# nikopj/FluxMPI.jl

Hardware: AMD Instinct MI355X
Metric: images/sec ResNet50 Lux.jl DDP at 1/2/4/8 MI355X; scaling efficiency (higher is better)
Workload: dtype bf16; 1 GPU; model=ResNet50, global_batch=256, per_gpu_batch=256, image_size=224, parallelism=dp1, optimizer=adam, conv=hybrid, norm=fused, memory_format=channels_last, backend=rccl, miopen_find=True, hip_graph=False, tunableop=False, kernel_choices=shipped, loss_finite=True, communicate=False

## Files before the change

csrc/api.h:

```cpp
#pragma once
#include <hip/hip_runtime.h>
#include <cstdint>
#include <vector>

namespace fluxmpi {

void mt_copy(const std::vector<uintptr_t>& src, const std::vector<uintptr_t>& dst,
             const std::vector<int64_t>& numel, int in_dtype, int out_dtype, double scale,
             hipStream_t stream);

void mt_fill(const std::vector<uintptr_t>& dst, const std::vector<int64_t>& numel, int dtype,
             double value, hipStream_t stream);

void mt_sumsq(const std::vector<uintptr_t>& src, const std::vector<int64_t>& numel, int dtype,
              float* out, hipStream_t stream);

struct SrHyper {
  uint64_t seed;
  uint32_t stream;
  uint32_t step;
  const uint32_t* dev_step;
  const int64_t* offsets = nullptr;
  size_t n_offsets = 0;
};
// ... 187 lines not shown
  const void* res;
  int64_t ldr;
  const void* bnb_x;
  const float* bnb_w;
  const float* bnb_b;
  const float* bnb_mean;
  const float* bnb_inv;
  const uint8_t* bnb_mask;
  int bnb_rm;
  int conv_h = 0, conv_w = 0, conv_c = 0;
  int engine = 0;
  const uint8_t* res_mask = nullptr;
  int res_sub_h = 0, res_sub_w = 0;
  int a_sub_h = 0, a_sub_w = 0;
  int conv_s = 1;
};
void gemm_bf16(const GemmProblem& g, hipStream_t stream);
void conv3bn3_bwd(const GemmProblem& g, hipStream_t stream);
void conv3ds_bwd(const void* dy, const uint8_t* relu_mask, const void* c3, const void* cds, const float* w,
                 const float* save_mean, const float* save_invstd, const float* sum_dy, const float* sum_dy_xhat,
                 const float* w2, const float* save_mean2, const float* save_invstd2, const float* sum_dy2,
                 const float* sum_dy_xhat2, const void* a2, const void* x, const void* wt3, const void* wtds,
                 void* d_a2, void* d_xside, float* ws3, float* wsds, int64_t P, int slabs, hipStream_t stream);
bool gemm_glds_supported(const GemmProblem& g);
void gemm_glds(const GemmProblem& g, hipStream_t stream);
void gemm_wgrad(const void* a, const void* b, float* ws, int64_t lda, int64_t ldb, int64_t M, int64_t N, int64_t K,
                int splits, int conv_h, int conv_w, int conv_c, hipStream_t stream, int variant = 0, int b_sub = 0);
void transpose_filters(const std::vector<uintptr_t>& src, const std::vector<uintptr_t>& dst,
                       const std::vector<int>& co, const std::vector<int>& ci, const std::vector<int>& taps,
                       hipStream_t stream);
void gemm_splitk_reduce(const float* ws, int splits, int64_t n, void* out, int out_dtype, hipStream_t stream);
void gemm_splitk_reduce_seg(const float* ws, int splits, int64_t n, int64_t seg, void* out0, void* out1, void* out2,
                            int out_dtype, hipStream_t stream);
bool wgrad256_supported(int64_t M, int64_t N, int64_t K, int64_t lda, int64_t ldb);
int wgrad256_actual_splits(int64_t K, int splits);
void wgrad256_set_variant(int v);
void gemm_wgrad256(const void* a, const void* b, float* ws, int64_t lda, int64_t ldb, int64_t M, int64_t N, int64_t K,
                   int splits, hipStream_t stream);
bool gemm_nt_supported(int64_t M, int64_t N, int64_t K, int64_t lda, int64_t ldb, int64_t ldc);
bool gemm_nt_conv_supported(int64_t pixels, int64_t C, int64_t Cout);
int gemm_nt_colpart_rows(int64_t M);
void gemm_nt_set_split(int min_ktiles);
int gemm_nt_get_split();
void gemm_nt(const void* a, const void* b, void* c, void* c2, const void* bias, int bias_f32, const void* h,
             float* colpart, float* stats, int64_t lda, int64_t ldb, int64_t ldc, int64_t M, int64_t N, int64_t K,
             int epi, hipStream_t stream);
// ... 67 lines not shown
```

csrc/bindings.cpp:

```cpp
#include <array>
#include <type_traits>
#include <pybind11/pybind11.h>
#include <pybind11/stl.h>

#include "api.h"
#include "comm/rccl_comm.h"

namespace py = pybind11;
using namespace fluxmpi;

template <typename T> using Py = std::conditional_t<std::is_pointer_v<T>, uintptr_t, T>;

template <typename T> T ptr(Py<T> v) {
  if constexpr (std::is_pointer_v<T>) return reinterpret_cast<T>(v);
  else return v;
}

template <typename T> std::array<T, 3> ptr3(const std::array<uintptr_t, 3>& v) {
  return {ptr<T>(v[0]), ptr<T>(v[1]), ptr<T>(v[2])};
}

template <typename R, typename... A> auto raw(R (*fn)(A...)) {
  return [fn](Py<A>... a) -> R { return fn(ptr<A>(a)...); };
}
// ... 107 lines not shown
PYBIND11_MODULE(_C_sr, m) {
  m.doc() = "fluxmpi_amd native library: stochastic rounding of the fused optimisers' bf16 stores";
  m.def("mt_adam", with_sr(&py_mt_adam), ADAM_ARGS, NO_SKIP, SR_ARGS);
  m.def("mt_sgd", with_sr(&py_mt_sgd), SGD_ARGS, NO_SKIP, SR_ARGS);
  m.def("mt_rule", with_sr(&py_mt_rule), RULE_ARGS, NO_SKIP, SR_ARGS);
  m.def(
      "mt_stochastic_round",
      [](Ptrs dst, Ptrs src, const std::vector<int64_t>& numel, uintptr_t dev_skip, uintptr_t stream, uint64_t seed,
         uint32_t sr_stream, uint32_t step, uintptr_t dev_step, const std::vector<int64_t>& offsets) {
        mt_stochastic_round(dst, src, numel, sr_hyper(seed, sr_stream, step, dev_step, offsets),
                            ptr<const int32_t*>(dev_skip), ptr<hipStream_t>(stream));
      },
      py::arg("dst"), py::arg("src"), py::arg("numel"), py::arg("dev_skip"), py::arg("stream"), SR_ARGS);
  m.def("sr_advance", raw(&sr_advance), py::arg("block"), py::arg("dev_skip"), py::arg("stream"));
}

PYBIND11_MODULE(_C_c3ds, m) {
  m.doc() = "fluxmpi_amd native library: one-pass backward around the dual BatchNorm of a downsample block";
  m.def("conv3ds_bwd", raw(&conv3ds_bwd), py::arg("dy"), py::arg("mask"), py::arg("c3"), py::arg("cds"), py::arg("w"),
        py::arg("mean"), py::arg("inv"), py::arg("sum_dy"), py::arg("sum_dy_xhat"), py::arg("w2"), py::arg("mean2"),
        py::arg("inv2"), py::arg("sum_dy2"), py::arg("sum_dy_xhat2"), py::arg("a2"), py::arg("x"), py::arg("wt3"),
        py::arg("wtds"), py::arg("d_a2"), py::arg("d_xside"), py::arg("ws3"), py::arg("wsds"), py::arg("P"),
        py::arg("slabs"), py::arg("stream"));
}

PYBIND11_MODULE(_C_aug, m) {
  m.doc() = "fluxmpi_amd native library: crop, flip, normalise, mixup / cutmix of a uint8 batch in one pass";
  m.def(
      "augment_batch",
      [](uintptr_t in, uintptr_t out, int64_t B, int H, int W, int h, int w, int C, int dtype, uint64_t seed,
         uint32_t aug_stream, uint32_t step, int64_t sample_offset, int mode, std::array<int, 4> box, float lam, int pad,
         int fill, int crop_center, int flip, std::array<float, 3> a, std::array<float, 3> b, uintptr_t dev_block,
         uintptr_t stream) {
        AugHyper hy{seed, aug_stream, step, sample_offset, mode, box[0], box[1], box[2], box[3], lam, pad, fill,
                    crop_center, flip, {a[0], a[1], a[2]}, {b[0], b[1], b[2]}, ptr<const uint32_t*>(dev_block)};
        augment_batch(ptr<const void*>(in), ptr<void*>(out), B, H, W, h, w, C, dtype, hy, ptr<hipStream_t>(stream));
      },
      py::arg("input"), py::arg("out"), py::arg("B"), py::arg("H"), py::arg("W"), py::arg("h"), py::arg("w"),
      py::arg("C"), py::arg("dtype"), py::arg("seed"), py::arg("aug_stream"), py::arg("step"),
      py::arg("sample_offset"), py::arg("mode"), py::arg("box"), py::arg("lam"), py::arg("pad"), py::arg("fill"),
      py::arg("crop_center"), py::arg("flip"), py::arg("a"), py::arg("b"), py::arg("dev_block"), py::arg("stream"));
  m.def(
      "aug_block_set",
      [](uintptr_t block, uint32_t step, int mode, std::array<int, 4> box, float lam, uintptr_t stream) {
        aug_block_set(ptr<void*>(block), step, mode, box[0], box[1], box[2], box[3], lam, ptr<hipStream_t>(stream));
      },
// ... 207 lines not shown
```

fluxmpi_amd/_build.py:

```python
from __future__ import annotations

import concurrent.futures as cf
import glob
import os
import re
import shutil
import subprocess
import sys
import sysconfig

ROOT = os.path.dirname(os.path.dirname(os.path.abspath(__file__)))
CSRC = os.path.join(ROOT, "csrc")
BUILD = os.path.join(ROOT, "build", "native")
ROCM = os.environ.get("ROCM_PATH", "/opt/rocm")
ARCH = os.environ.get("FLUXMPI_ARCH", "gfx950")


def _ext_suffix() -> str:
    return sysconfig.get_config_var("EXT_SUFFIX") or ".so"


def output_path() -> str:
    return os.path.join(ROOT, "fluxmpi_amd", "_C" + _ext_suffix())

# ... 9 lines not shown


def _torch_lib() -> str:
    import importlib.util

    spec = importlib.util.find_spec("torch")
    return os.path.join(os.path.dirname(spec.origin), "lib")


def _tool(name: str) -> str:
    for cand in (os.path.join(ROCM, "bin", name), os.path.join(ROCM, "llvm", "bin", name), shutil.which(name)):
        if cand and os.path.exists(cand):
            return cand
    raise FileNotFoundError(f"{name} not found (ROCM_PATH={ROCM})")


def _obj_for(src: str) -> str:
    rel = os.path.relpath(src, CSRC).replace(os.sep, "__")
    return os.path.join(BUILD, rel + ".o")


_NO_SLP = ["-fno-slp-vectorize"]
EXTRA_FLAGS = {f: _NO_SLP for f in ("gemm_nt.hip", "attention.hip", "gemm_glds.hip", "gemm.hip", "conv3x3n.hip",
                                        "wgrad3x3n.hip", "linbwd.hip", "conv3bn3_bwd.hip", "conv3ds_bwd.hip")}


NO_SCRATCH = ("conv3bn3_bwd.hip", "conv3ds_bwd.hip")


def _check_no_scratch(src: str, remarks: str) -> None:
    sizes = [int(m) for m in re.findall(r"ScratchSize \[bytes/lane\]: (\d+)", remarks)]
    if not sizes:
        raise RuntimeError(f"{src}: the compiler printed no kernel resource usage to check for scratch")
    if any(sizes):
        raise RuntimeError(f"{src}: a kernel spills to scratch ({max(sizes)} bytes/lane); it must not\n{remarks}")


def _compile_cmd(src: str, obj: str) -> list[str]:
    import pybind11

    common = ["-O3", "-fPIC", "-std=c++17", "-I", CSRC, "-Wall", "-Wno-unused-function",
              "-Wno-unused-variable", "-Wno-unused-but-set-variable"]
    if src.endswith(".hip"):
        return [_tool("hipcc"), f"--offload-arch={ARCH}", "-c", src, "-o", obj, *common,
                "-munsafe-fp-atomics", *EXTRA_FLAGS.get(os.path.basename(src), []),
                *(["-Rpass-analysis=kernel-resource-usage"] if os.path.basename(src) in NO_SCRATCH else [])]
    inc = [f"-I{pybind11.get_include()}", f"-I{sysconfig.get_paths()['include']}", f"-I{ROCM}/include"]
    return [_tool("amdclang++"), "-D__HIP_PLATFORM_AMD__=1", "-c", src, "-o", obj, *common, *inc,
            "-fvisibility=hidden"]

# ... 54 lines not shown
```

fluxmpi_amd/models/resnet.py:

```python
from __future__ import annotations

import os

import torch
import torch.nn as nn
import torch.nn.functional as F

from ..ops.linear import Linear

STEM = os.environ.get("FLUXMPI_STEM", "ours")


class Conv1x1(nn.Module):

    def __init__(self, cin: int, cout: int, stride: int = 1):
        super().__init__()
        self.stride = stride
        self.weight = nn.Parameter(torch.empty(cout, cin, 1, 1))
        nn.init.kaiming_normal_(self.weight, mode="fan_out", nonlinearity="relu")

    def forward(self, x):
        if self.stride != 1:
            x = x[:, :, ::self.stride, ::self.stride]
        n, c, h, w = x.shape
# ... 87 lines not shown
                    c1 = fb.conv1x1_stats(x, self.conv1.weight, link)
                    a1 = fb.bn_from_stats(c1, self.bn1, relu=True)
                cds = None
                c3ds = False
                if self.downsample is None:
                    identity = x
                elif fused_ds:
                    ds = self.downsample
                    dual = fb.dual_bn_ok(x, ds[0].out_channels, self.bn3, ds[1])
                    ds_stats = dual and fb.ds_forward_is_ours(x, ds[0].weight, ds[0].stride[0])
                    c3ds = self.hybrid and fb.conv3ds_ok(x, self.conv2, self.conv3, self.bn3, ds[0], ds[1])
                    identity = None
                    if not c3ds:
                        identity = fb.conv1x1_downsample(x, ds[0].weight, ds[0].stride[0],
                                                         link if isinstance(link, fb.SideGradLink) else None,
                                                         ours_stats=ds_stats)
                        if dual:
                            cds, identity = identity, None
                        else:
                            identity = ds[1](identity)
                else:
                    identity = self.downsample(x)
                if self.hybrid:
                    if fb.conv3x3_supported(a1, self.conv2):
                        ours = fb.conv3x3_forward_is_ours(a1, self.conv2.weight)
                        c2 = fb.conv3x3(a1, self.conv2.weight, with_stats=True)
                        a2 = fb.bn_from_stats(c2, self.bn2, relu=True, stats_ready=ours)
                    elif fb.conv3x3_s2_supported(a1, self.conv2):
                        ours = fb.conv3x3_s2_forward_is_ours(a1, self.conv2.weight)
                        c2 = fb.conv3x3_s2(a1, self.conv2.weight, with_stats=ours)
                        a2 = fb.bn_from_stats(c2, self.bn2, relu=True, stats_ready=ours)
                    else:
                        a2 = self.bn2(self.conv2(a1), relu=True)
                    o3 = fb.conv1x1_forward_is_ours(a2, self.conv3.weight)
                    if self.downsample is None and fb.conv3bn3_ok(a2, self.conv3, self.bn3, identity, link):
                        return fb.conv3_bn3_relu(a2, self.conv3, self.bn3, identity, link, ours_fwd=o3)
                    if c3ds:
                        return fb.conv3ds_bn_relu(a2, self.conv3, self.bn3, x, ds[0], ds[1], link, ours3=o3,
                                                  ours_ds=ds_stats)
                    c3 = fb.conv1x1_hybrid(a2, self.conv3.weight, None, ours_stats=o3)
                else:
                    c2 = fb.conv3x3(a1, self.conv2.weight) if fb.conv3x3_supported(a1, self.conv2) else self.conv2(a1)
                    c3 = fb.bn_relu_conv1x1(c2, self.bn2, self.conv3.weight)
                if cds is not None:
                    out = fb.dual_bn_relu(c3, self.bn3, cds, self.downsample[1],
                                          stats_ready=o3 if self.hybrid else True, ds_stats_ready=ds_stats)
                elif self.hybrid and not o3:
                    out = self.bn3(c3, relu=True, residual=identity, link=link if self.downsample is None else None)
                elif self.hybrid:
                    out = fb.bn_from_stats(c3, self.bn3, relu=True, residual=identity, stats_ready=True,
                                           link=link if self.downsample is None else None)
                else:
                    out = fb.bn_from_stats(c3, self.bn3, relu=True, residual=identity,
                                           link=link if self.downsample is None else None)
                return out
        identity = x if self.downsample is None else self.downsample(x)
        if self.fused:
            out = self.bn1(self.conv1(x), relu=True)
            out = self.bn2(self.conv2(out), relu=True)
            return self.bn3(self.conv3(out), relu=True, residual=identity)
        out = F.relu(self.bn1(self.conv1(x)))
        out = F.relu(self.bn2(self.conv2(out)))
        out = self.bn3(self.conv3(out))
# ... 94 lines not shown
```

fluxmpi_amd/ops/_ext.py:

```python
from __future__ import annotations

import importlib
import importlib.util
import os

import torch

from ..utils.errors import NativeExtensionError

_MOD = None
_TRIED = False
_ERR: Exception | None = None


def _try_import():
    global _MOD, _TRIED, _ERR
    if _TRIED:
        return _MOD
    _TRIED = True
    try:
        _MOD = importlib.import_module("fluxmpi_amd._C")
    except Exception as e:
        _MOD = None
        _ERR = e
# ... 39 lines not shown
            raise NativeExtensionError(
                f"fluxmpi_amd.{name} ({what} of {C.__file__}) failed to load: {e!r}. "
                "Rebuild: `python -c 'import fluxmpi_amd; fluxmpi_amd.build()'`.") from e
        _EXTRA[name] = mod
    return _EXTRA[name]


def scale():
    return _extra("_C_scale", "the loss-scaling entries")


def ema():
    return _extra("_C_ema", "the weight-EMA entries")


def sr():
    return _extra("_C_sr", "the stochastic-rounding entries")


def c3ds():
    return _extra("_C_c3ds", "the downsample-block backward entry")


def aug():
    return _extra("_C_aug", "the input-pipeline entries")


def require_for(t: torch.Tensor):
    if t.is_cuda:
        return get(required=True)
    return None
```

fluxmpi_amd/ops/batchnorm.py:

```python
from __future__ import annotations

import torch
import torch.nn as nn
import torch.nn.functional as F

from . import _ext
from . import graddst
from ._launch import nhwc, ptr, stream
from .multi_tensor import DTYPE_CODE


def _rows_c(x: torch.Tensor):
    if x.dim() == 4:
        n, c, h, w = x.shape
        return n * h * w, c
    if x.dim() == 2:
        return x.shape[0], x.shape[1]
    raise ValueError("fused batchnorm expects 2D [N,C] or 4D [N,C,H,W] input")


_nhwc = nhwc


_SHARDS = 64
# ... 110 lines not shown



def launch_finalize(x, w32, b32, running_mean, running_var, momentum, eps, nbt, pending, ws=None, affine=False):
    rows, ch = _rows_c(x)
    out = [torch.empty(ch, device=x.device, dtype=torch.float32) for _ in range(4 if affine else 2)]
    mean, inv, scale, shift = out if affine else (*out, None, None)
    ws = _workspace(x) if ws is None else ws
    _ext.get(required=True).bn_stats_finalize(
        x.data_ptr(), w32.data_ptr(), b32.data_ptr(), ptr(running_mean), ptr(running_var), mean.data_ptr(),
        inv.data_ptr(), ptr(scale), ptr(shift), ws.data_ptr(), rows, ch, float(momentum), float(eps), int(pending),
        DTYPE_CODE[x.dtype], stream(x), ptr(nbt))
    return out


def launch_apply(x, w32, b32, mean, inv, relu, residual=None):
    rows, ch = _rows_c(x)
    res = nhwc(residual) if residual is not None else None
    y = torch.empty_like(x)
    mask = torch.empty(x.numel() // 8, device=x.device, dtype=torch.uint8) if (relu and res is not None) else None
    _ext.get(required=True).bn_apply(x.data_ptr(), y.data_ptr(), ptr(res), ptr(w32), ptr(b32), mean.data_ptr(),
                                     inv.data_ptr(), rows, ch, int(relu), ptr(mask), DTYPE_CODE[x.dtype], stream(x))
    return y, mask


def launch_bwd(dy, x, mask, w32, b32, mean, inv, relu, want_dres=False, stats_ready=False, params=(None, None),
               want_dx=True):
    rows, ch = _rows_c(x)
    dx = torch.empty_like(x) if want_dx else None
    dres = torch.empty_like(x) if want_dres else None
    dw, db = (_grad_out(p, ch, x) for p in params)
    ws = _link_workspace(x) if stats_ready else _workspace(x)
    _ext.get(required=True).bn_bwd(dy.data_ptr(), x.data_ptr(), 0, ptr(mask), ptr(w32), ptr(b32), mean.data_ptr(),
                                   inv.data_ptr(), ptr(dx), ptr(dres), dw.data_ptr(), db.data_ptr(), ws.data_ptr(),
                                   rows, ch, int(relu), DTYPE_CODE[x.dtype], stream(x), int(stats_ready))
    return dx, dres, dw, db


def launch_bwd_dual(dy, mask, c3, cds, w32, mean, inv, w232, mean2, inv2, params, want_dx=True):
    rows, ch = _rows_c(c3)
    dx, dx2 = (torch.empty_like(c3), torch.empty_like(cds)) if want_dx else (None, None)
    dw, db, dw2, db2 = (_grad_out(p, ch, c3) for p in params)
    _ext.get(required=True).bn_bwd_dual(
        dy.data_ptr(), mask.data_ptr(), c3.data_ptr(), cds.data_ptr(), w32.data_ptr(), mean.data_ptr(),
        inv.data_ptr(), w232.data_ptr(), mean2.data_ptr(), inv2.data_ptr(), ptr(dx), ptr(dx2), dw.data_ptr(),
        db.data_ptr(), dw2.data_ptr(), db2.data_ptr(), _workspace(c3).data_ptr(), _dual_workspace(c3).data_ptr(), rows,
# ... 114 lines not shown
```

fluxmpi_amd/ops/fused_block.py:

```python
from __future__ import annotations

import os

import torch

from . import _ext
from . import graddst
from ._launch import conv_backward, nhwc, stream as _stream
from .batchnorm import (BNStatsLink, GradLink, SideGradLink, _dual_workspace, _link_workspace,
                        _workspace, bn_counter, finish_bwd, hands_masked, launch_apply, launch_bwd, launch_bwd_dual,
                        launch_finalize)
from . import gemm as G
from . import gemm_nt as _NT
from . import groupnorm as _GN
from .conv_choice import (_DGRAD_CHOICE, _DS_CHOICE, _FWD1_CHOICE, _FWD_CHOICE, _FWD_ENGINE, _S2_CHOICE,
                          _WG_CHOICE, FWD_ENGINES, choices_frozen, dump_choices, freeze_choices,
                          load_choice_lines, load_choices, no_measure as _no_measure, stats_choice,
                          time_us as _time_us, w256_ok as _w256_ok, w3n_configs, wgrad_best)
from .gemm import conv1x1_dgrad, conv1x1_wgrad, conv3x3_dgrad, conv3x3_fwd, gemm, note_filter
from .multi_tensor import DTYPE_CODE


CONV3X3 = "ours"
CONV1X1 = "ours"
DUAL_BN = True
DS_FWD = "ours"
DS_WGRAD = True
S2_FWD = True


def _nhwc2d(x: torch.Tensor) -> torch.Tensor:
    x = nhwc(x)
    n, c, h, w = x.shape
    return x.permute(0, 2, 3, 1).reshape(n * h * w, c)
# ... 76 lines not shown
    if link is not None:
        g = link.take()
        if isinstance(g, tuple):
            res, res_mask = _nhwc2d(g[0]), g[1]
        elif isinstance(g, Stride2Grad):
            res, res_sub = _nhwc2d(g.t), (h, w)
        elif g is not None:
            res = _nhwc2d(g)
    bn = stats = None
    if bnlink is not None and bnlink.bound and bnlink.x.shape == x.shape and \
            bnlink.x.is_contiguous(memory_format=torch.channels_last):
        bn = (_nhwc2d(bnlink.x), bnlink.w32, bnlink.b32, bnlink.mean, bnlink.inv, bnlink.mask, bnlink.relu_mode)
        stats = _link_workspace(dx)
    conv1x1_dgrad(dc2, weight.reshape(co, ci), residual=res, out=_nhwc2d(dx), bn_bwd=bn, stats=stats, w4d=weight,
                  residual_mask=res_mask, residual_sub=res_sub)
    if bn is not None:
        bnlink.ready = True
    return dx


class _Conv1x1Hybrid(torch.autograd.Function):

    @staticmethod
    def forward(ctx, x, weight, link=None, bnlink=None, ours_stats=False):
        x = nhwc(x)
        ctx.link, ctx.bnlink = link, bnlink
        note_filter(weight)
        ctx.save_for_backward(x, weight)
        if ours_stats:
            return _fwd1x1_stats(x, weight, _workspace(x))
        return torch.nn.functional.conv2d(x, weight)

    @staticmethod
    def backward(ctx, dc):
        x, weight = ctx.saved_tensors
        dc = nhwc(dc)
        dw = None
        if ctx.needs_input_grad[1]:
            dw = wgrad_best(("1x1", tuple(x.shape), weight.shape[0]), _wgrad1x1_candidates(dc, x, weight), param=weight)
        dx = _dgrad_nhwc(_nhwc2d(dc), weight, x, ctx.link, ctx.bnlink) if ctx.needs_input_grad[0] else None
        return dx, dw, None, None, None


def _ds_fwd_ours(x, weight, stride, stats):
    n, ci, h, w = x.shape
    co = weight.shape[0]
    ho, wo = (h + stride - 1) // stride, (w + stride - 1) // stride
    c = _empty_nhwc(n, co, ho, wo, x)
    gemm(_nhwc2d(x), weight.reshape(co, ci), c, M=n * ho * wo, N=co, K=ci, lda=ci, ldb=ci, ldc=co, mode=1,
         stats=stats, a_sub=(h, w) if stride == 2 else None)
    return c


def ds_forward_supported(x, weight, stride) -> bool:
    return (DS_FWD in ("ours", "force") and G.ENGINE != 1 and x.is_cuda and x.dtype == torch.bfloat16 and x.dim() == 4
            and weight.dtype == torch.bfloat16 and stride in (1, 2) and x.shape[1] % 8 == 0
            and weight.shape[0] % 8 == 0 and x.numel() // x.shape[1] < 2 ** 31)


def ds_forward_is_ours(x, weight, stride) -> bool:
    if not ds_forward_supported(x, weight, stride):
        return False
    if DS_FWD == "force":
        return True
# ... 77 lines not shown
        ctx.relu, ctx.has_res, ctx.wdtype = relu, residual is not None, weight.dtype
        ctx.params = (weight, bias)
        ctx.link = link if residual is not None else None
        ctx.bnlink = bnlink
        if bnlink is not None:
            bnlink.bind(x, *saved, relu)
        ctx.save_for_backward(x, *saved)
        return y

    @staticmethod
    def backward(ctx, dy):
        x, mask, w32, b32, mean, inv = ctx.saved_tensors
        dy = nhwc(dy)
        ready = ctx.bnlink is not None and ctx.bnlink.ready
        hand_masked = hands_masked(ctx.link, mask, ctx.relu)
        dx, dres, dw, db = launch_bwd(dy, x, mask, w32, b32, mean, inv, ctx.relu, ctx.has_res and not hand_masked,
                                      ready, ctx.params)
        if ctx.bnlink is not None:
            ctx.bnlink.release()
        dw, db, dres = finish_bwd(dw, db, ctx.wdtype, True, True, ctx.link, dy, mask, dres, hand_masked)
        return dx, dw, db, dres, None, None, None, None, None, None, None, None, None


class _Conv3BN3(torch.autograd.Function):

    @staticmethod
    def forward(ctx, a2, weight, bn_weight, bn_bias, residual, running_mean, running_var, momentum, eps, nbt, link,
                ours_fwd):
        a2 = nhwc(a2)
        note_filter(weight)
        c3 = _fwd1x1_stats(a2, weight, _workspace(a2)) if ours_fwd else torch.nn.functional.conv2d(a2, weight)
        y, saved = _bn_fwd_from_stats(c3, bn_weight, bn_bias, residual, running_mean, running_var, momentum, eps, True,
                                      ours_fwd, nbt)
        ctx.link, ctx.wdtype, ctx.params = link, bn_weight.dtype, (bn_weight, bn_bias)
        ctx.save_for_backward(a2, weight, c3, *saved)
        return y

    @staticmethod
    def backward(ctx, dy):
        a2, weight, c3, mask, w32, b32, mean, inv = ctx.saved_tensors
        dy = nhwc(dy)
        n, ci, h, w = a2.shape
        _, _, dbw, dbb = launch_bwd(dy, c3, mask, w32, b32, mean, inv, True, params=ctx.params, want_dx=False)
        part = torch.empty(conv3bn3_slabs(n * h * w, dy.device), weight.shape[0], ci, device=dy.device,
                           dtype=torch.float32)
        d_a2 = _one_pass_branch(dy, mask, c3, w32, mean, inv, (dbb, dbw), a2, weight, part, _empty_nhwc(n, ci, h, w, a2))
        dw = _slabs_to_wgrad(part, weight) if ctx.needs_input_grad[1] else None
        dbw, dbb, _ = finish_bwd(dbw, dbb, ctx.wdtype, True, True, ctx.link, dy, mask, None, True)
        return (d_a2, dw, dbw, dbb, None, None, None, None, None, None, None, None)


def _one_pass_branch(dy, mask, c, w32, mean, inv, sums, act, weight, part, out):
    co, ci = weight.shape[0], weight.shape[1]
    return gemm(dy, weight, out, M=act.numel() // ci, N=ci, K=co, lda=co, ldb=ci, ldc=ci, a_kmajor=True, b_kmajor=False,
                mode=4, splits=part.shape[0], a_affine=sums, stats=part, residual=_nhwc2d(act),
                bn_bwd=(c, w32, None, mean, inv, mask, 3))


def _slabs_to_wgrad(part, weight):
    co, ci = weight.shape[0], weight.shape[1]
    with graddst.into(weight):
        dw = graddst.empty((co, ci), weight.dtype, part.device)
    _ext.get(required=True).gemm_splitk_reduce(part.data_ptr(), part.shape[0], co * ci, dw.data_ptr(),
                                               DTYPE_CODE[dw.dtype], _stream(part))
    return dw.view(co, ci, 1, 1)


CONV3BN3 = os.environ.get("FLUXMPI_CONV3BN3", "1") != "0"


def conv3bn3_slabs(rows: int, device) -> int:
    cus = torch.cuda.get_device_properties(device).multi_processor_count
    return max(1, min(-(-rows // 32), 2 * cus))


def _fused_bn_training(*bns) -> bool:
    from .batchnorm import FusedBatchNorm2d
    return all(isinstance(m, FusedBatchNorm2d) and m.training and m.affine and m.track_running_stats for m in bns)


def conv3bn3_ok(a2, conv, bn, residual, link) -> bool:
    wt = conv.weight
    return (CONV3BN3 and G.ENGINE != 1 and a2.is_cuda and a2.dim() == 4 and a2.dtype == torch.bfloat16
            and wt.dtype == torch.bfloat16 and tuple(wt.shape) == (256, 64, 1, 1) and wt.is_contiguous()
            and a2.shape[1] == 64 and a2.numel() // 64 < 2 ** 31 and residual is not None
            and residual.shape == (a2.shape[0], 256, a2.shape[2], a2.shape[3]) and residual.dtype == a2.dtype
            and (link.masked if link is not None else not (residual.requires_grad and torch.is_grad_enabled()))
            and _fused_bn_training(bn))


def conv3_bn3_relu(a2, conv, bn, residual, link=None, ours_fwd=True):
    mom, nbt = bn_counter(bn)
    return _Conv3BN3.apply(a2, conv.weight, bn.weight, bn.bias, residual, bn.running_mean, bn.running_var, mom,
                           bn.eps, nbt, link, bool(ours_fwd))


def _dual_bn_fwd(c3, bn, stats_ready, cds, bn2, ds_ready):
    w, b, rm, rv, mom, eps, nbt = bn
    w2, b2, rm2, rv2, mom2, eps2, nbt2 = bn2
    c3, cds = nhwc(c3), nhwc(cds)
    w32, b32, w232, b232 = w.float(), b.float(), w2.float(), b2.float()
    mean, inv = launch_finalize(c3, w32, b32, rm, rv, mom, eps, nbt, stats_ready)
    mean2, inv2 = launch_finalize(cds, w232, b232, rm2, rv2, mom2, eps2, nbt2, ds_ready,
                                  ws=_dual_workspace(c3) if ds_ready else None)
    ch = c3.shape[1]
    y = torch.empty_like(c3)
    mask = torch.empty(c3.numel() // 8, device=c3.device, dtype=torch.uint8)
    _ext.get(required=True).bn_apply_dual(
        c3.data_ptr(), cds.data_ptr(), y.data_ptr(), w32.data_ptr(), b32.data_ptr(), mean.data_ptr(), inv.data_ptr(),
        w232.data_ptr(), b232.data_ptr(), mean2.data_ptr(), inv2.data_ptr(), c3.numel() // ch, ch, mask.data_ptr(),
        DTYPE_CODE[c3.dtype], _stream(c3))
    return y, (c3, cds, mask, w32, mean, inv, w232, mean2, inv2)


class _DualBN(torch.autograd.Function):

    @staticmethod
# ... 20 lines not shown
    from .batchnorm import kernel_supported
    ch = c.shape[1]
    return (DUAL_BN and kernel_supported(c) and c.dim() == 4 and (ch & (ch - 1)) == 0
            and _fused_bn_training(bn, bn_ds))


def dual_bn_relu(c3, bn, cds, bn_ds, stats_ready=False, ds_stats_ready=False):
    mom, nbt = bn_counter(bn)
    mom2, nbt2 = bn_counter(bn_ds)
    return _DualBN.apply(c3, bn.weight, bn.bias, bn.running_mean, bn.running_var, mom, bn.eps, nbt, stats_ready,
                         cds, bn_ds.weight, bn_ds.bias, bn_ds.running_mean, bn_ds.running_var, mom2, bn_ds.eps, nbt2,
                         ds_stats_ready)


def dual_bn_ok(x, ch, bn, bn_ds) -> bool:
    return (DUAL_BN and x.is_cuda and x.dtype in (torch.bfloat16, torch.float16, torch.float32) and x.dim() == 4
            and ch % 8 == 0 and 8 <= ch <= 2048 and (ch & (ch - 1)) == 0 and _fused_bn_training(bn, bn_ds))


class _Conv3DsBN(torch.autograd.Function):

    @staticmethod
    def forward(ctx, a2, w3, x, wds, w, b, w2, b2, rm, rv, mom, eps, nbt, rm2, rv2, mom2, eps2, nbt2, link, ours3,
                ours_ds, form):
        a2, x = nhwc(a2), nhwc(x)
        note_filter(w3)
        note_filter(wds)
        c3 = _fwd1x1_stats(a2, w3, _workspace(a2)) if ours3 else torch.nn.functional.conv2d(a2, w3)
        cds = _ds_fwd_ours(x, wds, 1, _dual_workspace(x)) if ours_ds else torch.nn.functional.conv2d(x, wds)
        y, saved = _dual_bn_fwd(c3, (w, b, rm, rv, mom, eps, nbt), ours3, cds, (w2, b2, rm2, rv2, mom2, eps2, nbt2),
                                ours_ds)
        ctx.link, ctx.form = link, form
        ctx.wdtypes = (w.dtype, w2.dtype)
        ctx.params = (w, b, w2, b2)
        ctx.save_for_backward(a2, w3, x, wds, *saved)
        return y

    @staticmethod
    def backward(ctx, dy):
        a2, w3, x, wds, c3, cds, mask, w32, mean, inv, w232, mean2, inv2 = ctx.saved_tensors
        dy = nhwc(dy)
        n, ci, h, w = a2.shape
        co, rows = w3.shape[0], n * h * w
        dev = dy.device
        _, _, dw, db, dw2, db2 = launch_bwd_dual(dy, mask, c3, cds, w32, mean, inv, w232, mean2, inv2, ctx.params,
                                                 want_dx=False)
        d_a2, d_x = _empty_nhwc(n, ci, h, w, a2), _empty_nhwc(n, ci, h, w, x)
        if ctx.form == 2:
            slabs = conv3ds_slabs(rows, dev)
            part = torch.empty(2, slabs, co, ci, device=dev, dtype=torch.float32)
            _ext.c3ds().conv3ds_bwd(dy.data_ptr(), mask.data_ptr(), c3.data_ptr(), cds.data_ptr(), w32.data_ptr(),
                                    mean.data_ptr(), inv.data_ptr(), db.data_ptr(), dw.data_ptr(), w232.data_ptr(),
                                    mean2.data_ptr(), inv2.data_ptr(), db2.data_ptr(), dw2.data_ptr(), a2.data_ptr(),
                                    x.data_ptr(), w3.data_ptr(), wds.data_ptr(), d_a2.data_ptr(), d_x.data_ptr(),
                                    part[0].data_ptr(), part[1].data_ptr(), rows, slabs, _stream(dy))
        else:
            part = torch.empty(2, conv3bn3_slabs(rows, dev), co, ci, device=dev, dtype=torch.float32)
            _one_pass_branch(dy, mask, c3, w32, mean, inv, (db, dw), a2, w3, part[0], d_a2)
            _one_pass_branch(dy, mask, cds, w232, mean2, inv2, (db2, dw2), x, wds, part[1], d_x)
        grads = [_slabs_to_wgrad(part[i], wt) if ctx.needs_input_grad[1 + 2 * i] else None
                 for i, wt in enumerate((w3, wds))]
        if ctx.link is not None and ctx.link.offer(d_x):
            d_x = None
        t1, t2 = ctx.wdtypes
        return (d_a2, grads[0], d_x, grads[1], dw.to(t1), db.to(t1), dw2.to(t2), db2.to(t2)) + (None,) * 14


CONV3DS = int(os.environ.get("FLUXMPI_CONV3DS", "1"))


def conv3ds_slabs(rows: int, device) -> int:
    cus = torch.cuda.get_device_properties(device).multi_processor_count
    return max(1, min(-(-rows // 32), cus))


def conv3ds_ok(x, conv2, conv3, bn, ds_conv, bn_ds) -> bool:
    w3, wds = conv3.weight, ds_conv.weight
    return (CONV3DS in (1, 2) and G.ENGINE != 1 and x.is_cuda and x.dim() == 4 and x.dtype == torch.bfloat16
            and x.shape[1] == 64 and x.is_contiguous(memory_format=torch.channels_last)
            and x.numel() < 2 ** 31 and tuple(conv2.stride) == (1, 1) and tuple(ds_conv.stride) == (1, 1)
            and all(wt.dtype == torch.bfloat16 and tuple(wt.shape) == (256, 64, 1, 1) and wt.is_contiguous()
                    for wt in (w3, wds))
            and dual_bn_ok(x, 256, bn, bn_ds))


def conv3ds_bn_relu(a2, conv3, bn, x, ds_conv, bn_ds, link=None, ours3=True, ours_ds=True):
    mom, nbt = bn_counter(bn)
    mom2, nbt2 = bn_counter(bn_ds)
    return _Conv3DsBN.apply(a2, conv3.weight, x, ds_conv.weight, bn.weight, bn.bias, bn_ds.weight, bn_ds.bias,
                            bn.running_mean, bn.running_var, mom, bn.eps, nbt, bn_ds.running_mean, bn_ds.running_var,
                            mom2, bn_ds.eps, nbt2, link, bool(ours3), bool(ours_ds), CONV3DS)


class _BNReluConv1x1(torch.autograd.Function):

    @staticmethod
    def forward(ctx, c2, bn_weight, bn_bias, running_mean, running_var, weight, momentum, eps, nbt=None,
                stats_ready=False):
        c2 = nhwc(c2)
        n, ch, h, w = c2.shape
        w32, b32 = bn_weight.float(), bn_bias.float()
        mean, inv, scale, shift = launch_finalize(c2, w32, b32, running_mean, running_var, momentum, eps, nbt,
                                                  stats_ready, affine=True)
        co = weight.shape[0]
        c3 = _empty_nhwc(n, co, h, w, c2)
        gemm(_nhwc2d(c2), weight.reshape(co, ch), c3, M=n * h * w, N=co, K=ch, lda=ch, ldb=ch, ldc=co, a_kmajor=True,
             b_kmajor=True, mode=1, stats=_workspace(c2), a_affine=(scale, shift))
        ctx.bn_wdtype = bn_weight.dtype
        ctx.params = (bn_weight, bn_bias)
        ctx.save_for_backward(c2, w32, b32, mean, inv, scale, shift, weight)
        return c3

    @staticmethod
    def backward(ctx, dc3):
# ... 191 lines not shown
    return dx + residual if residual is not None else dx


def masked_links_ok() -> bool:
    return G.ENGINE != 1


def conv1x1_stats(x, weight, link=None, bnlink=None):
    return _Conv1x1Stats.apply(x, weight, link, bnlink)


def conv1x1_forward_is_ours(x, weight) -> bool:
    if CONV1X1 != "ours":
        return False
    def make():
        xs, w = x.detach().contiguous(memory_format=torch.channels_last), weight.detach()
        n, _, h, wd = xs.shape
        ws = torch.zeros_like(_workspace(xs))
        return (lambda: _fwd1x1_stats(xs, w, ws), lambda: torch.nn.functional.conv2d(xs, w),
                n * h * wd * w.shape[0] * xs.element_size())
    return stats_choice(_FWD1_CHOICE, (tuple(x.shape), weight.shape[0]), make)


def conv1x1_hybrid(x, weight, link=None, bnlink=None, ours_stats=False):
    return _Conv1x1Hybrid.apply(x, weight, link, bnlink, ours_stats)


def bn_from_stats(x, bn, relu=False, residual=None, stats_ready=True, link=None, bnlink=None):
    mom, nbt = bn_counter(bn)
    return _BNFromStats.apply(x, bn.weight, bn.bias, residual, bn.running_mean, bn.running_var, mom, bn.eps, relu,
                              stats_ready, link, nbt, bnlink)


def bn_relu_conv1x1(c2, bn, weight, stats_ready=False):
    mom, nbt = bn_counter(bn)
    return _BNReluConv1x1.apply(c2, bn.weight, bn.bias, bn.running_mean, bn.running_var, weight, mom, bn.eps, nbt,
                                stats_ready)


def supported(x: torch.Tensor, *channels: int) -> bool:
    return (x.is_cuda and x.dtype == torch.bfloat16 and x.dim() == 4
            and all(c % 32 == 0 and 32 <= c <= 2048 for c in channels))
```

Measured before the change: 13090 images/s.

## Fuse bn2 apply, ReLU and conv3 1x1 forward with stats into one kernel

```diff
diff --git a/csrc/api.h b/csrc/api.h
--- a/csrc/api.h
+++ b/csrc/api.h
@@ -233,6 +233,9 @@
                  const float* w2, const float* save_mean2, const float* save_invstd2, const float* sum_dy2,
                  const float* sum_dy_xhat2, const void* a2, const void* x, const void* wt3, const void* wtds,
                  void* d_a2, void* d_xside, float* ws3, float* wsds, int64_t P, int slabs, hipStream_t stream);
+bool bn_relu_conv1x1_fwd_supported(int Cin, int Cout);
+void bn_relu_conv1x1_fwd(const void* c2, const float* scale, const float* shift, const void* wt, void* a2, void* c3,
+                         float* stats, int64_t P, int Cin, int Cout, hipStream_t stream);
 bool gemm_glds_supported(const GemmProblem& g);
 void gemm_glds(const GemmProblem& g, hipStream_t stream);
 void gemm_wgrad(const void* a, const void* b, float* ws, int64_t lda, int64_t ldb, int64_t M, int64_t N, int64_t K,
diff --git a/csrc/bindings.cpp b/csrc/bindings.cpp
--- a/csrc/bindings.cpp
+++ b/csrc/bindings.cpp
@@ -153,6 +153,14 @@
         py::arg("inv2"), py::arg("sum_dy2"), py::arg("sum_dy_xhat2"), py::arg("a2"), py::arg("x"), py::arg("wt3"),
         py::arg("wtds"), py::arg("d_a2"), py::arg("d_xside"), py::arg("ws3"), py::arg("wsds"), py::arg("P"),
         py::arg("slabs"), py::arg("stream"));
+}
+
+PYBIND11_MODULE(_C_bn2c3, m) {
+  m.doc() = "fluxmpi_amd native library: BatchNorm apply + ReLU + 1x1 expansion convolution forward";
+  m.def("bn_relu_conv1x1_fwd_supported", &bn_relu_conv1x1_fwd_supported, py::arg("Cin"), py::arg("Cout"));
+  m.def("bn_relu_conv1x1_fwd", raw(&bn_relu_conv1x1_fwd), py::arg("c2"), py::arg("scale"), py::arg("shift"),
+        py::arg("wt"), py::arg("a2"), py::arg("c3"), py::arg("stats"), py::arg("P"), py::arg("Cin"), py::arg("Cout"),
+        py::arg("stream"));
 }
 
 PYBIND11_MODULE(_C_aug, m) {
diff --git a/csrc/kernels/bn_relu_conv1x1_fwd.hip b/csrc/kernels/bn_relu_conv1x1_fwd.hip
--- /dev/null
+++ b/csrc/kernels/bn_relu_conv1x1_fwd.hip
@@ -0,0 +1,213 @@
+#include <stdexcept>
+#include <string>
+
+#include "../api.h"
+#include "c3_frag.h"
+#include "common.h"
+
+namespace fluxmpi {
+namespace {
+
+constexpr int kTP = 32;
+constexpr int kShards = 64;
+
+template <int CIN>
+struct Cfg {
+  static constexpr int kCo = 4 * CIN;
+  static constexpr int kWaves = kCo / 64;
+  static constexpr int kThreads = 64 * kWaves;
+  static constexpr int kVecIn = CIN / 8, kVecOut = kCo / 8;
+  static constexpr int kLdA = CIN + 8, kLdC = kCo + 8;
+  static constexpr int kKS = CIN / 32;
+  static constexpr int kRpp = kThreads / kVecOut;
+  static constexpr int kPasses = kTP / kRpp;
+  static_assert(kThreads * 8 == kTP * CIN, "one c2 vector per lane and tile");
+  static_assert(kThreads % kVecIn == 0 && kThreads % kVecOut == 0, "a lane keeps its channels across tiles");
+  static_assert(kThreads == kCo, "one lane per column issues the atomics");
+  static_assert(kRpp * 2 * kCo * 4 <= kTP * kLdC * 2, "the final reduction reuses the staging tile");
+};
+
+struct Args {
+  const bf16* c2;
+  const float* scale;
+  const float* shift;
+  const bf16* wt;
+  bf16* a2;
+  bf16* c3;
+  float* stats;
+  int64_t P;
+};
+
+template <int CIN, int MINW>
+__global__ __launch_bounds__(Cfg<CIN>::kThreads, MINW) void bn_relu_conv1x1_fwd_kernel(Args p) {
+  using C = Cfg<CIN>;
+  constexpr int kCo = C::kCo;
+  __shared__ __attribute__((aligned(16))) bf16 atile[kTP * C::kLdA];
+  __shared__ __attribute__((aligned(16))) bf16 ctile[kTP * C::kLdC];
+  __shared__ __attribute__((aligned(16))) float ksm[2 * CIN];
+  const int t = threadIdx.x;
+  const int wave = __builtin_amdgcn_readfirstlane(t >> 6), lane = t & 63;
+  const int row = t / C::kVecIn, cv = t % C::kVecIn;
+  const int orow = t / C::kVecOut, ov = t % C::kVecOut;
+  const int64_t ntiles = (p.P + kTP - 1) / kTP;
+
+  for (int c = t; c < CIN; c += C::kThreads) {
+    const int slot = ((c >> 2) & 1) * (CIN / 2) + (c >> 3) * 4 + (c & 3);
+    ksm[slot] = p.scale[c];
+    ksm[CIN + slot] = p.shift[c];
+  }
+  bf16x8 wf[4][C::kKS];
+#pragma unroll
+  for (int j = 0; j < 4; ++j)
+#pragma unroll
+    for (int ks = 0; ks < C::kKS; ++ks)
+      wf[j][ks] = *reinterpret_cast<const bf16x8*>(p.wt + (64 * wave + 16 * j + (lane & 15)) * CIN + 32 * ks +
+                                                   8 * (lane >> 4));
+  __syncthreads();
+
+  uint4 qc;
+  auto issue = [&](int64_t tl) {
+    const int64_t p0 = tl * kTP;
+    const int nr = p.P - p0 < kTP ? static_cast<int>(p.P - p0) : kTP;
+    const int r = row < nr ? row : nr - 1;
+    qc = reinterpret_cast<const uint4*>(p.c2 + p0 * CIN)[static_cast<unsigned>(r) * C::kVecIn + cv];
+  };
+
+  float s[8], q[8];
+#pragma unroll
+  for (int j = 0; j < 8; ++j) s[j] = q[j] = 0.f;
+
+  int64_t tl = blockIdx.x;
+  if (tl < ntiles) issue(tl);
+  for (; tl < ntiles; tl += gridDim.x) {
+    const int64_t p0 = tl * kTP;
+    const int nr = p.P - p0 < kTP ? static_cast<int>(p.P - p0) : kTP;
+    int opq = 0;
+    asm volatile("" : "+v"(opq));
+    const float4* kl = reinterpret_cast<const float4*>(ksm + opq) + cv;
+    float sc[8], sh[8];
+#pragma unroll
+    for (int hf = 0; hf < 2; ++hf) {
+      const float4 ka = kl[hf * (CIN / 8)], kb = kl[(CIN / 4) + hf * (CIN / 8)];
+      sc[4 * hf + 0] = ka.x; sc[4 * hf + 1] = ka.y; sc[4 * hf + 2] = ka.z; sc[4 * hf + 3] = ka.w;
+      sh[4 * hf + 0] = kb.x; sh[4 * hf + 1] = kb.y; sh[4 * hf + 2] = kb.z; sh[4 * hf + 3] = kb.w;
+    }
+    {
+      bf16 tx[8];
+      __builtin_memcpy(tx, &qc, 16);
+      const bool ok = row < nr;
+      bf16x8 o;
+#pragma unroll
+      for (int j = 0; j < 8; ++j) {
+        float f = fmaf(static_cast<float>(tx[j]), sc[j], sh[j]);
+        f = f > 0.f ? f : 0.f;
+        o[j] = ok ? static_cast<bf16>(f) : static_cast<bf16>(0.f);
+      }
+      *reinterpret_cast<bf16x8*>(atile + row * C::kLdA + cv * 8) = o;
+      if (ok) *reinterpret_cast<bf16x8*>(p.a2 + p0 * CIN + static_cast<unsigned>(row * CIN + cv * 8)) = o;
+    }
+    __syncthreads();
+    if (tl + gridDim.x < ntiles) issue(tl + gridDim.x);
+
+    {
+      const bf16* brow = atile + (lane & 15) * C::kLdA + 8 * (lane >> 4);
+      bf16* crow = ctile + (lane & 15) * C::kLdC + 64 * wave + 4 * (lane >> 4);
+#pragma unroll
+      for (int i = 0; i < kTP / 16; ++i) {
+        f32x4 acc[4];
+#pragma unroll
+        for (int j = 0; j < 4; ++j) acc[j] = f32x4{0.f, 0.f, 0.f, 0.f};
+        bf16x8 fb = *reinterpret_cast<const bf16x8*>(brow + 16 * i * C::kLdA);
+#pragma unroll
+        for (int ks = 0; ks < C::kKS; ++ks) {
+          bf16x8 fn = fb;
+          if (ks + 1 < C::kKS) fn = *reinterpret_cast<const bf16x8*>(brow + 16 * i * C::kLdA + 32 * (ks + 1));
+#pragma unroll
+          for (int j = 0; j < 4; ++j) acc[j] = __builtin_amdgcn_mfma_f32_16x16x32_bf16(wf[j][ks], fb, acc[j], 0, 0, 0);
+          __builtin_amdgcn_sched_barrier(0);
+          fb = fn;
+        }
+#pragma unroll
+        for (int j = 0; j < 4; ++j) {
+          bf16x4 o;
+#pragma unroll
+          for (int r = 0; r < 4; ++r) o[r] = static_cast<bf16>(acc[j][r]);
+          *reinterpret_cast<bf16x4*>(crow + 16 * i * C::kLdC + 16 * j) = o;
+        }
+        __builtin_amdgcn_sched_barrier(0);
+      }
+    }
+    __syncthreads();
+    {
+      const bf16* cb = ctile + orow * C::kLdC + ov * 8;
+      const unsigned oo = static_cast<unsigned>(orow * kCo + ov * 8);
+#pragma unroll
+      for (int ps = 0; ps < C::kPasses; ++ps) {
+        const bf16x8 v = *reinterpret_cast<const bf16x8*>(cb + C::kRpp * ps * C::kLdC);
+        bf16* ob = p.c3 + (p0 + C::kRpp * ps) * kCo;
+#pragma unroll
+        for (int j = 0; j < 8; ++j) {
+          const float f = static_cast<float>(v[j]);
+          s[j] += f;
+          q[j] = fmaf(f, f, q[j]);
+        }
+        if (orow < nr - C::kRpp * ps) *reinterpret_cast<bf16x8*>(ob + oo) = v;
+      }
+    }
+  }
+
+  __syncthreads();
+  float* red = reinterpret_cast<float*>(ctile);
+#pragma unroll
+  for (int hf = 0; hf < 2; ++hf) {
+    *reinterpret_cast<float4*>(red + (orow * 2 + 0) * kCo + ov * 8 + 4 * hf) =
+        float4{s[4 * hf], s[4 * hf + 1], s[4 * hf + 2], s[4 * hf + 3]};
+    *reinterpret_cast<float4*>(red + (orow * 2 + 1) * kCo + ov * 8 + 4 * hf) =
+        float4{q[4 * hf], q[4 * hf + 1], q[4 * hf + 2], q[4 * hf + 3]};
+  }
+  __syncthreads();
+  float ts = 0.f, tq = 0.f;
+#pragma unroll
+  for (int g = 0; g < C::kRpp; ++g) {
+    ts += red[(g * 2 + 0) * kCo + t];
+    tq += red[(g * 2 + 1) * kCo + t];
+  }
+  float* shard = p.stats + static_cast<size_t>(blockIdx.x % kShards) * 2 * kCo;
+  atomicAdd(shard + t, ts);
+  atomicAdd(shard + kCo + t, tq);
+}
+
+template <int CIN, int MINW>
+void launch(const Args& a, hipStream_t stream) {
+  using C = Cfg<CIN>;
+  auto k = bn_relu_conv1x1_fwd_kernel<CIN, MINW>;
+  const int64_t ntiles = (a.P + kTP - 1) / kTP;
+  const int64_t slots = resident_blocks(reinterpret_cast<const void*>(k), C::kThreads, 0);
+  k<<<static_cast<unsigned>(ntiles < slots ? ntiles : slots), C::kThreads, 0, stream>>>(a);
+  FLUXMPI_HIP_CHECK(hipGetLastError());
+}
+
+}
+
+bool bn_relu_conv1x1_fwd_supported(int Cin, int Cout) { return (Cin == 64 && Cout == 256) || (Cin == 128 && Cout == 512); }
+
+void bn_relu_conv1x1_fwd(const void* c2, const float* scale, const float* shift, const void* wt, void* a2, void* c3,
+                         float* stats, int64_t P, int Cin, int Cout, hipStream_t stream) {
+  if (!bn_relu_conv1x1_fwd_supported(Cin, Cout) || P < 1 || P > (INT64_MAX >> 12))
+    throw std::runtime_error("bn_relu_conv1x1_fwd: needs (Cin, Cout) = (64, 256) or (128, 512) and P >= 1; got P=" +
+                             std::to_string(P) + ", Cin=" + std::to_string(Cin) + ", Cout=" + std::to_string(Cout));
+  if (c2 == nullptr || scale == nullptr || shift == nullptr || wt == nullptr || a2 == nullptr || c3 == nullptr ||
+      stats == nullptr)
+    throw std::runtime_error("bn_relu_conv1x1_fwd: c2, scale, shift, W, a2, c3 and the statistics workspace are all required");
+  uintptr_t bits = 0;
+  for (const void* q : {c2, static_cast<const void*>(scale), static_cast<const void*>(shift), wt,
+                        static_cast<const void*>(a2), static_cast<const void*>(c3), static_cast<const void*>(stats)})
+    bits |= reinterpret_cast<uintptr_t>(q);
+  if ((bits & 15u) != 0) throw std::runtime_error("bn_relu_conv1x1_fwd: operands must be 16-byte aligned");
+  const Args a{static_cast<const bf16*>(c2), scale, shift, static_cast<const bf16*>(wt), static_cast<bf16*>(a2),
+               static_cast<bf16*>(c3), stats, P};
+  if (Cin == 64) launch<64, 2>(a, stream);
+  else launch<128, 4>(a, stream);
+}
+
+}
diff --git a/fluxmpi_amd/_build.py b/fluxmpi_amd/_build.py
--- a/fluxmpi_amd/_build.py
+++ b/fluxmpi_amd/_build.py
@@ -55,10 +55,11 @@
 
 _NO_SLP = ["-fno-slp-vectorize"]
 EXTRA_FLAGS = {f: _NO_SLP for f in ("gemm_nt.hip", "attention.hip", "gemm_glds.hip", "gemm.hip", "conv3x3n.hip",
-                                        "wgrad3x3n.hip", "linbwd.hip", "conv3bn3_bwd.hip", "conv3ds_bwd.hip")}
+                                        "wgrad3x3n.hip", "linbwd.hip", "conv3bn3_bwd.hip", "conv3ds_bwd.hip",
+                                        "bn_relu_conv1x1_fwd.hip")}
 
 
-NO_SCRATCH = ("conv3bn3_bwd.hip", "conv3ds_bwd.hip")
+NO_SCRATCH = ("conv3bn3_bwd.hip", "conv3ds_bwd.hip", "bn_relu_conv1x1_fwd.hip")
 
 
 def _check_no_scratch(src: str, remarks: str) -> None:
diff --git a/fluxmpi_amd/models/resnet.py b/fluxmpi_amd/models/resnet.py
--- a/fluxmpi_amd/models/resnet.py
+++ b/fluxmpi_amd/models/resnet.py
@@ -133,23 +133,27 @@
                 else:
                     identity = self.downsample(x)
                 if self.hybrid:
+                    c2 = None
                     if fb.conv3x3_supported(a1, self.conv2):
                         ours = fb.conv3x3_forward_is_ours(a1, self.conv2.weight)
                         c2 = fb.conv3x3(a1, self.conv2.weight, with_stats=True)
-                        a2 = fb.bn_from_stats(c2, self.bn2, relu=True, stats_ready=ours)
                     elif fb.conv3x3_s2_supported(a1, self.conv2):
                         ours = fb.conv3x3_s2_forward_is_ours(a1, self.conv2.weight)
                         c2 = fb.conv3x3_s2(a1, self.conv2.weight, with_stats=ours)
+                    c3 = None
+                    if c2 is None:
+                        a2 = self.bn2(self.conv2(a1), relu=True)
+                    elif fb.bn2conv3_ok(c2, self.bn2, self.conv3):
+                        a2, c3 = fb.bn_relu_conv3(c2, self.bn2, self.conv3, stats_ready=ours)
+                    else:
                         a2 = fb.bn_from_stats(c2, self.bn2, relu=True, stats_ready=ours)
-                    else:
-                        a2 = self.bn2(self.conv2(a1), relu=True)
-                    o3 = fb.conv1x1_forward_is_ours(a2, self.conv3.weight)
+                    o3 = c3 is not None or fb.conv1x1_forward_is_ours(a2, self.conv3.weight)
                     if self.downsample is None and fb.conv3bn3_ok(a2, self.conv3, self.bn3, identity, link):
-                        return fb.conv3_bn3_relu(a2, self.conv3, self.bn3, identity, link, ours_fwd=o3)
+                        return fb.conv3_bn3_relu(a2, self.conv3, self.bn3, identity, link, ours_fwd=o3, c3=c3)
                     if c3ds:
                         return fb.conv3ds_bn_relu(a2, self.conv3, self.bn3, x, ds[0], ds[1], link, ours3=o3,
-                                                  ours_ds=ds_stats)
-                    c3 = fb.conv1x1_hybrid(a2, self.conv3.weight, None, ours_stats=o3)
+                                                  ours_ds=ds_stats, c3=c3)
+                    c3 = fb.conv1x1_hybrid(a2, self.conv3.weight, None, ours_stats=o3, c=c3)
                 else:
                     c2 = fb.conv3x3(a1, self.conv2.weight) if fb.conv3x3_supported(a1, self.conv2) else self.conv2(a1)
                     c3 = fb.bn_relu_conv1x1(c2, self.bn2, self.conv3.weight)
diff --git a/fluxmpi_amd/ops/_ext.py b/fluxmpi_amd/ops/_ext.py
--- a/fluxmpi_amd/ops/_ext.py
+++ b/fluxmpi_amd/ops/_ext.py
@@ -85,6 +85,10 @@
     return _extra("_C_c3ds", "the downsample-block backward entry")
 
 
+def bn2c3():
+    return _extra("_C_bn2c3", "the bn2 + conv3 forward entry")
+
+
 def aug():
     return _extra("_C_aug", "the input-pipeline entries")
 
diff --git a/fluxmpi_amd/ops/batchnorm.py b/fluxmpi_amd/ops/batchnorm.py
--- a/fluxmpi_amd/ops/batchnorm.py
+++ b/fluxmpi_amd/ops/batchnorm.py
@@ -156,6 +156,17 @@
     _ext.get(required=True).bn_apply(x.data_ptr(), y.data_ptr(), ptr(res), ptr(w32), ptr(b32), mean.data_ptr(),
                                      inv.data_ptr(), rows, ch, int(relu), ptr(mask), DTYPE_CODE[x.dtype], stream(x))
     return y, mask
+
+
+def launch_apply_conv1x1(x, scale, shift, weight, ws=None):
+    n, ch, h, w = x.shape
+    co = weight.shape[0]
+    y = torch.empty_like(x)
+    c = torch.empty(n, h, w, co, device=x.device, dtype=x.dtype).permute(0, 3, 1, 2)
+    ws = _workspace(x) if ws is None else ws
+    _ext.bn2c3().bn_relu_conv1x1_fwd(x.data_ptr(), scale.data_ptr(), shift.data_ptr(), weight.data_ptr(), y.data_ptr(),
+                                     c.data_ptr(), ws.data_ptr(), n * h * w, ch, co, stream(x))
+    return y, c
 
 
 def launch_bwd(dy, x, mask, w32, b32, mean, inv, relu, want_dres=False, stats_ready=False, params=(None, None),
diff --git a/fluxmpi_amd/ops/fused_block.py b/fluxmpi_amd/ops/fused_block.py
--- a/fluxmpi_amd/ops/fused_block.py
+++ b/fluxmpi_amd/ops/fused_block.py
@@ -8,8 +8,8 @@
 from . import graddst
 from ._launch import conv_backward, nhwc, stream as _stream
 from .batchnorm import (BNStatsLink, GradLink, SideGradLink, _dual_workspace, _link_workspace,
-                        _workspace, bn_counter, finish_bwd, hands_masked, launch_apply, launch_bwd, launch_bwd_dual,
-                        launch_finalize)
+                        _workspace, bn_counter, finish_bwd, hands_masked, launch_apply, launch_apply_conv1x1, launch_bwd,
+                        launch_bwd_dual, launch_finalize)
 from . import gemm as G
 from . import gemm_nt as _NT
 from . import groupnorm as _GN
@@ -132,11 +132,13 @@
 class _Conv1x1Hybrid(torch.autograd.Function):
 
     @staticmethod
-    def forward(ctx, x, weight, link=None, bnlink=None, ours_stats=False):
+    def forward(ctx, x, weight, link=None, bnlink=None, ours_stats=False, c=None):
         x = nhwc(x)
         ctx.link, ctx.bnlink = link, bnlink
         note_filter(weight)
         ctx.save_for_backward(x, weight)
+        if c is not None:
+            return c
         if ours_stats:
             return _fwd1x1_stats(x, weight, _workspace(x))
         return torch.nn.functional.conv2d(x, weight)
@@ -149,7 +151,7 @@
         if ctx.needs_input_grad[1]:
             dw = wgrad_best(("1x1", tuple(x.shape), weight.shape[0]), _wgrad1x1_candidates(dc, x, weight), param=weight)
         dx = _dgrad_nhwc(_nhwc2d(dc), weight, x, ctx.link, ctx.bnlink) if ctx.needs_input_grad[0] else None
-        return dx, dw, None, None, None
+        return dx, dw, None, None, None, None
 
 
 def _ds_fwd_ours(x, weight, stride, stats):
@@ -273,14 +275,62 @@
         return dx, dw, db, dres, None, None, None, None, None, None, None, None, None
 
 
+class _BN2Conv3(torch.autograd.Function):
+
+    @staticmethod
+    def forward(ctx, c2, weight, bias, running_mean, running_var, momentum, eps, stats_ready, nbt, conv_weight):
+        c2 = nhwc(c2)
+        w32, b32 = weight.float(), bias.float()
+        mean, inv, scale, shift = launch_finalize(c2, w32, b32, running_mean, running_var, momentum, eps, nbt,
+                                                  stats_ready, affine=True)
+        a2, c3 = launch_apply_conv1x1(c2, scale, shift, conv_weight)
+        ctx.wdtype, ctx.params = weight.dtype, (weight, bias)
+        ctx.save_for_backward(c2, w32, b32, mean, inv)
+        ctx.mark_non_differentiable(c3)
+        ctx.set_materialize_grads(False)
+        return a2, c3
+
+    @staticmethod
+    def backward(ctx, dy, _):
+        if dy is None:
+            return (None,) * 10
+        c2, w32, b32, mean, inv = ctx.saved_tensors
+        dx, _, dw, db = launch_bwd(nhwc(dy), c2, None, w32, b32, mean, inv, True, params=ctx.params)
+        dw, db, _ = finish_bwd(dw, db, ctx.wdtype, True, True, None, None, None, None, False)
+        return dx, dw, db, None, None, None, None, None, None, None
+
+
+BN2CONV3 = os.environ.get("FLUXMPI_BN2CONV3", "1") != "0"
+
+
+def bn2conv3_ok(c2, bn, conv) -> bool:
+    wt = conv.weight
+    if not (BN2CONV3 and G.ENGINE != 1 and torch.is_grad_enabled() and c2.is_cuda and c2.dim() == 4
+            and c2.dtype == torch.bfloat16 and c2.is_contiguous(memory_format=torch.channels_last)
+            and wt.dtype == torch.bfloat16 and wt.is_contiguous()
+            and (c2.shape[1], tuple(wt.shape)) in ((64, (256, 64, 1, 1)), (128, (512, 128, 1, 1)))
+            and _fused_bn_training(bn)):
+        return False
+    cus = torch.cuda.get_device_properties(c2.device).multi_processor_count
+    return c2.numel() // c2.shape[1] >= 32 * 2 * cus and conv1x1_forward_is_ours(c2, wt)
+
+
+def bn_relu_conv3(c2, bn, conv, stats_ready=True):
+    mom, nbt = bn_counter(bn)
+    return _BN2Conv3.apply(c2, bn.weight, bn.bias, bn.running_mean, bn.running_var, mom, bn.eps, stats_ready, nbt,
+                           conv.weight)
+
+
 class _Conv3BN3(torch.autograd.Function):
 
     @staticmethod
     def forward(ctx, a2, weight, bn_weight, bn_bias, residual, running_mean, running_var, momentum, eps, nbt, link,
-                ours_fwd):
+                ours_fwd, c3=None):
         a2 = nhwc(a2)
         note_filter(weight)
-        c3 = _fwd1x1_stats(a2, weight, _workspace(a2)) if ours_fwd else torch.nn.functional.conv2d(a2, weight)
+        ours_fwd = ours_fwd or c3 is not None
+        if c3 is None:
+            c3 = _fwd1x1_stats(a2, weight, _workspace(a2)) if ours_fwd else torch.nn.functional.conv2d(a2, weight)
         y, saved = _bn_fwd_from_stats(c3, bn_weight, bn_bias, residual, running_mean, running_var, momentum, eps, True,
                                       ours_fwd, nbt)
         ctx.link, ctx.wdtype, ctx.params = link, bn_weight.dtype, (bn_weight, bn_bias)
@@ -298,7 +348,7 @@
         d_a2 = _one_pass_branch(dy, mask, c3, w32, mean, inv, (dbb, dbw), a2, weight, part, _empty_nhwc(n, ci, h, w, a2))
         dw = _slabs_to_wgrad(part, weight) if ctx.needs_input_grad[1] else None
         dbw, dbb, _ = finish_bwd(dbw, dbb, ctx.wdtype, True, True, ctx.link, dy, mask, None, True)
-        return (d_a2, dw, dbw, dbb, None, None, None, None, None, None, None, None)
+        return (d_a2, dw, dbw, dbb, None, None, None, None, None, None, None, None, None)
 
 
 def _one_pass_branch(dy, mask, c, w32, mean, inv, sums, act, weight, part, out):
@@ -340,10 +390,10 @@
             and _fused_bn_training(bn))
 
 
-def conv3_bn3_relu(a2, conv, bn, residual, link=None, ours_fwd=True):
+def conv3_bn3_relu(a2, conv, bn, residual, link=None, ours_fwd=True, c3=None):
     mom, nbt = bn_counter(bn)
     return _Conv3BN3.apply(a2, conv.weight, bn.weight, bn.bias, residual, bn.running_mean, bn.running_var, mom,
-                           bn.eps, nbt, link, bool(ours_fwd))
+                           bn.eps, nbt, link, bool(ours_fwd), c3)
 
 
 def _dual_bn_fwd(c3, bn, stats_ready, cds, bn2, ds_ready):
@@ -410,11 +460,13 @@
 
     @staticmethod
     def forward(ctx, a2, w3, x, wds, w, b, w2, b2, rm, rv, mom, eps, nbt, rm2, rv2, mom2, eps2, nbt2, link, ours3,
-                ours_ds, form):
+                ours_ds, form, c3=None):
         a2, x = nhwc(a2), nhwc(x)
         note_filter(w3)
         note_filter(wds)
-        c3 = _fwd1x1_stats(a2, w3, _workspace(a2)) if ours3 else torch.nn.functional.conv2d(a2, w3)
+        ours3 = ours3 or c3 is not None
+        if c3 is None:
+            c3 = _fwd1x1_stats(a2, w3, _workspace(a2)) if ours3 else torch.nn.functional.conv2d(a2, w3)
         cds = _ds_fwd_ours(x, wds, 1, _dual_workspace(x)) if ours_ds else torch.nn.functional.conv2d(x, wds)
         y, saved = _dual_bn_fwd(c3, (w, b, rm, rv, mom, eps, nbt), ours3, cds, (w2, b2, rm2, rv2, mom2, eps2, nbt2),
                                 ours_ds)
@@ -451,7 +503,7 @@
         if ctx.link is not None and ctx.link.offer(d_x):
             d_x = None
         t1, t2 = ctx.wdtypes
-        return (d_a2, grads[0], d_x, grads[1], dw.to(t1), db.to(t1), dw2.to(t2), db2.to(t2)) + (None,) * 14
+        return (d_a2, grads[0], d_x, grads[1], dw.to(t1), db.to(t1), dw2.to(t2), db2.to(t2)) + (None,) * 15
 
 
 CONV3DS = int(os.environ.get("FLUXMPI_CONV3DS", "1"))
@@ -472,12 +524,12 @@
             and dual_bn_ok(x, 256, bn, bn_ds))
 
 
-def conv3ds_bn_relu(a2, conv3, bn, x, ds_conv, bn_ds, link=None, ours3=True, ours_ds=True):
+def conv3ds_bn_relu(a2, conv3, bn, x, ds_conv, bn_ds, link=None, ours3=True, ours_ds=True, c3=None):
     mom, nbt = bn_counter(bn)
     mom2, nbt2 = bn_counter(bn_ds)
     return _Conv3DsBN.apply(a2, conv3.weight, x, ds_conv.weight, bn.weight, bn.bias, bn_ds.weight, bn_ds.bias,
                             bn.running_mean, bn.running_var, mom, bn.eps, nbt, bn_ds.running_mean, bn_ds.running_var,
-                            mom2, bn_ds.eps, nbt2, link, bool(ours3), bool(ours_ds), CONV3DS)
+                            mom2, bn_ds.eps, nbt2, link, bool(ours3), bool(ours_ds), CONV3DS, c3)
 
 
 class _BNReluConv1x1(torch.autograd.Function):
@@ -715,8 +767,8 @@
     return stats_choice(_FWD1_CHOICE, (tuple(x.shape), weight.shape[0]), make)
 
 
-def conv1x1_hybrid(x, weight, link=None, bnlink=None, ours_stats=False):
-    return _Conv1x1Hybrid.apply(x, weight, link, bnlink, ours_stats)
+def conv1x1_hybrid(x, weight, link=None, bnlink=None, ours_stats=False, c=None):
+    return _Conv1x1Hybrid.apply(x, weight, link, bnlink, ours_stats, c)
 
 
 def bn_from_stats(x, bn, relu=False, residual=None, stats_ready=True, link=None, bnlink=None):
```

Result: faster. 13220 images/s, median of 6 (+1.0%).
